# jshi31/T2ONet

Hardware: AMD Instinct MI355X
Metric: images/sec (train step: episode forward + END select + L1 + backward + gradient all-reduce + Adam, bs=64/GPU, 256x256 fp32) (higher is better)
Workload: dtype f32; 1 GPU; BASELINE.json configs[2]: full T2ONet episode/L1 train step (train_seq2seqL1.py:74-88), bs=64 per GPU, 256x256 fp32, FiveK-shaped synthetic batch, random-init weights; global_batch=64, parallelism=dp1: batch shards, one flat fp32 gradient all-reduce (22.2 M floats) per step, world_size=1

## Files before the change

### include/t2onet_hip.h

```cpp
#ifndef T2ONET_HIP_H
#define T2ONET_HIP_H

#include <stddef.h>

#ifdef __cplusplus
extern "C" {
#endif

#define T2O_OK 0
#define T2O_EINVAL 1
#define T2O_EUNSUPPORTED 2
#define T2O_EWORKSPACE 3
#define T2O_ELAUNCH 4

#define T2O_OP_IDENTITY (-1)
#define T2O_MAX_PARAM 24

int t2o_abi_version(void);
const char* t2o_last_error(void);
const char* t2o_source_digest(void);

int t2o_op_num_params(int op);

size_t t2o_workspace_bytes(int B, int H, int W);
// ... 164 lines not shown


int t2o_bn_relu_nhwc_bwd_acc(const float* x, const float* y, const float* dy, const float* weight, const float* bias,
                             const float* save_mean, const float* save_invstd, float* dx, float* dres, float* dweight,
                             float* dbias, int has_res, int relu, int accumulate, void* workspace, size_t workspace_bytes,
                             int M, int C, void* stream);
int t2o_bn_relu_nhwc_bwd_partials_acc(const float* x, const float* dy, const float* weight, const float* bias,
                                      const float* save_mean, const float* save_invstd, float* dx, float* dweight,
                                      float* dbias, int relu, int accumulate, const float* partial, int partial_rows,
                                      void* workspace, size_t workspace_bytes, int M, int C, void* stream);

int t2o_conv3x3_wgrad_acc_nhwc(const float* x, const float* dy, float* dw, void* workspace, size_t workspace_bytes,
                               int N, int Ho, int Wo, int Ci, int Co, int stride, int accumulate, void* stream);

int t2o_conv_weight_transform(const float* w, float* wt, int Co, int Ci, int taps, int flip, void* stream);
int t2o_conv_weight_transform_batch(const float* const* w, float* const* wt, const int* Co, const int* Ci, const int* taps,
                                    const int* flip, int n, void* stream);

int t2o_conv3x3_dgrad_pre_nhwc(const float* dy, const float* wt, const float* addend, float* dx, void* workspace,
                               size_t workspace_bytes, int N, int H, int W, int Ci, int Co, void* stream);
int t2o_conv3x3_dgrad_bnsums_rows(int N, int H, int W, int Ci, int Co);
int t2o_conv3x3_dgrad_pre_bnsums_nhwc(const float* dy, const float* wt, float* dx, const float* bn_x,
                                      const float* save_mean, const float* save_invstd, const float* weight,
                                      const float* bias, float* rows, void* workspace, size_t workspace_bytes,
                                      int N, int H, int W, int Ci, int Co, void* stream);
int t2o_conv3x3s2_dgrad_pre_nhwc(const float* dy, const float* wt, float* dx, void* workspace, size_t workspace_bytes,
                                 int N, int Ho, int Wo, int Ci, int Co, void* stream);

int t2o_stem_fwd(const float* x, const float* w, float* y, float* stats, int N, int Ho, int Wo, int Co, int planar, void* stream);
int t2o_stem_fwd_any(const float* x, const float* w, float* y, float* stats, int N, int Hi, int Wi, int Co, int planar, void* stream);
int t2o_stem_wgrad(const float* x, const float* dy, float* dw, void* workspace, size_t workspace_bytes, int N, int Ho, int Wo,
                   int Co, int planar, int accumulate, void* stream);
int t2o_stem_dgrad(const float* dy, const float* w, float* dx, int N, int Ho, int Wo, int Co, int planar, int accumulate, void* stream);

int t2o_conv1x1s2_fwd_nhwc(const float* x, const float* w, float* y, int N, int H, int W, int Ci, int Co, void* stream);
int t2o_conv1x1s2_dgrad_acc_nhwc(const float* dy, const float* wt, float* dx, int N, int H, int W, int Ci, int Co, void* stream);
size_t t2o_conv1x1s2_wgrad_workspace_bytes(int N, int H, int W, int Ci, int Co);
int t2o_conv1x1s2_wgrad_nhwc(const float* x, const float* dy, float* dw, void* workspace, size_t workspace_bytes,
                             int N, int H, int W, int Ci, int Co, int accumulate, void* stream);

int t2o_conv3x3_any_fwd_nhwc(const float* x, const float* w, float* y, int N, int H, int W, int Ci, int Co, int stride, void* stream);
int t2o_conv3x3_any_dgrad_nhwc(const float* dy, const float* wt, const float* addend, float* dx, int N, int H, int W, int Ci, int Co,
                               int stride, void* stream);
size_t t2o_conv3x3_any_wgrad_workspace_bytes(int N, int H, int W, int Ci, int Co, int stride);
int t2o_conv3x3_any_wgrad_nhwc(const float* x, const float* dy, float* dw, void* workspace, size_t workspace_bytes,
                               int N, int H, int W, int Ci, int Co, int stride, int accumulate, void* stream);

int t2o_wino_padded_tiles(int N, int H, int W);
int t2o_wino_weight_transform(const float* w, float* U, int Cn, int Ck, void* stream);
int t2o_wino_weight_transform_batch(const float* const* w, float* const* U, const int* Cn, const int* Ck, int n, void* stream);
int t2o_wino_weight_transform_chunked_batch(const float* const* w, float* const* Uc, const int* Cn, const int* Ck, int n, void* stream);
int t2o_wino_input_transform(const float* x, float* V, int N, int H, int W, int C, void* stream);
int t2o_wino_input_transform_ld(const float* x, float* V, int N, int H, int W, int C, int plane_rows, void* stream);
int t2o_wino_stats_rows(int N, int H, int W, int C);
int t2o_wino_output_transform(const float* M, const float* addend, float* y, float* stats, int N, int H, int W, int C, void* stream);
int t2o_wino_dy_transform(const float* dy, float* Ad, int N, int H, int W, int C, void* stream);
int t2o_wino_dy_transforms(const float* dy, float* V, float* Ad, int N, int H, int W, int C, void* stream);
int t2o_wino_dy_transforms_ld(const float* dy, float* V, float* Ad, int N, int H, int W, int C, int ad_plane_rows, void* stream);
int t2o_wino_dy_transform_ld(const float* dy, float* Ad, int N, int H, int W, int C, int plane_rows, void* stream);
int t2o_wino_dw_transform(const float* dU, float* dw, int Co, int Ci, int splits, int accumulate, void* stream);
int t2o_gemm_nt_batched(const float* A, const float* B, float* C, int batches, int M, int N, int K, int a_rows, void* stream);
int t2o_gemm_tn_splits(int batches, int rows, int M, int N);
int t2o_gemm_tn_batched(const float* A, const float* B, float* C, int batches, int rows, int M, int N, int splits, void* stream);
int t2o_gemm_tn_batched_ld(const float* A, const float* B, float* C, int batches, int rows, int a_plane_rows, int b_plane_rows, int M, int N,
                           int splits, void* stream);

// ... 125 lines not shown
```

### t2onet_amd/_lib.py

```python
import ctypes
import os

import torch

_HERE = os.path.dirname(os.path.abspath(__file__))
LIB_PATH = os.path.join(_HERE, 'lib', 'libt2onet_hip.so')

c_f = ctypes.POINTER(ctypes.c_float)
c_i = ctypes.POINTER(ctypes.c_int)
_P = ctypes.c_void_p
_I = ctypes.c_int
_Z = ctypes.c_size_t
_F = ctypes.c_float
_D = ctypes.c_double

SIGNATURES = {
    't2o_abi_version': (_I, []),
    't2o_last_error': (ctypes.c_char_p, []),
    't2o_source_digest': (ctypes.c_char_p, []),
    't2o_op_num_params': (_I, [_I]),
    't2o_workspace_bytes': (_Z, [_I, _I, _I]),
    't2o_op_fwd': (_I, [_I, _P, _P, _I, _P, _I, _P, _I, _I, _I, _P]),
    't2o_op_bwd': (_I, [_I, _P, _P, _I, _P, _I, _P, _P, _P, _I, _P, _Z, _I, _I, _I, _P]),
    't2o_apply_fwd': (_I, [_P, _P, _P, _I, _P, _I, _P, _I, _I, _I, _P]),
# ... 69 lines not shown
    't2o_wino_weight_transform_chunked_batch': (_I, [_P, _P, _P, _P, _I, _P]),
    't2o_end_select_l1_fwd': (_I, [_P, _I, _P, _P, _P, _I, _Z, _P, _Z, _P]),
    't2o_end_select_l1_bwd': (_I, [_P, _P, _I, _P, _P, _P, _I, _Z, _P]),
    't2o_wino_padded_tiles': (_I, [_I, _I, _I]),
    't2o_wino_weight_transform': (_I, [_P, _P, _I, _I, _P]),
    't2o_gemm_nt_batched': (_I, [_P, _P, _P, _I, _I, _I, _I, _I, _P]),
    't2o_gemm': (_I, [_P, _P, _P, _I, _I, _I, _I, _I, _I, _I, _I, _I, _P]),
    't2o_colsum': (_I, [_P, _P, _I, _I, _I, _I, _P]),
    't2o_gemm_tn_splits': (_I, [_I, _I, _I, _I]),
    't2o_gemm_tn_batched': (_I, [_P, _P, _P, _I, _I, _I, _I, _I, _P]),
    't2o_gemm_tn_batched_ld': (_I, [_P, _P, _P, _I, _I, _I, _I, _I, _I, _I, _P]),
    't2o_wino_input_transform': (_I, [_P, _P, _I, _I, _I, _I, _P]),
    't2o_wino_input_transform_ld': (_I, [_P, _P, _I, _I, _I, _I, _I, _P]),
    't2o_wino_stats_rows': (_I, [_I, _I, _I, _I]),
    't2o_wino_output_transform': (_I, [_P, _P, _P, _P, _I, _I, _I, _I, _P]),
    't2o_wino_dy_transform': (_I, [_P, _P, _I, _I, _I, _I, _P]),
    't2o_wino_dy_transforms': (_I, [_P, _P, _P, _I, _I, _I, _I, _P]),
    't2o_wino_dy_transforms_ld': (_I, [_P, _P, _P, _I, _I, _I, _I, _I, _P]),
    't2o_wino_dy_transform_ld': (_I, [_P, _P, _I, _I, _I, _I, _I, _P]),
    't2o_wino_dw_transform': (_I, [_P, _P, _I, _I, _I, _I, _P]),
    't2o_conv3x3_dgrad_pre_nhwc': (_I, [_P, _P, _P, _P, _P, _Z, _I, _I, _I, _I, _I, _P]),
    't2o_conv3x3_dgrad_bnsums_rows': (_I, [_I, _I, _I, _I, _I]),
    't2o_wino_fused_supported': (_I, [_I, _I, _I, _I, _I]),
    't2o_wino_fused_stats_rows': (_I, [_I, _I, _I]),
    't2o_wino_u_chunked': (_I, [_P, _P, _I, _I, _P]),
    't2o_wino_fused_conv_nhwc': (_I, [_P, _P, _P, _P, _P, _P, _I, _I, _I, _I, _I, _P]),
    't2o_wino_fused_conv_bnsums_nhwc': (_I, [_P, _P, _P, _P, _P, _P, _P, _P, _P, _P, _I, _I, _I, _I, _I, _P]),
    't2o_conv3x3_dgrad_pre_bnsums_nhwc': (_I, [_P, _P, _P, _P, _P, _P, _P, _P, _P, _P, _Z, _I, _I, _I, _I, _I, _P]),
    't2o_conv3x3s2_dgrad_pre_nhwc': (_I, [_P, _P, _P, _P, _Z, _I, _I, _I, _I, _I, _P]),
    't2o_stem_fwd': (_I, [_P, _P, _P, _P, _I, _I, _I, _I, _I, _P]),
    't2o_stem_fwd_any': (_I, [_P, _P, _P, _P, _I, _I, _I, _I, _I, _P]),
    't2o_stem_wgrad': (_I, [_P, _P, _P, _P, _Z, _I, _I, _I, _I, _I, _I, _P]),
    't2o_stem_dgrad': (_I, [_P, _P, _P, _I, _I, _I, _I, _I, _I, _P]),
    't2o_conv1x1s2_fwd_nhwc': (_I, [_P, _P, _P, _I, _I, _I, _I, _I, _P]),
    't2o_conv1x1s2_dgrad_acc_nhwc': (_I, [_P, _P, _P, _I, _I, _I, _I, _I, _P]),
    't2o_conv1x1s2_wgrad_workspace_bytes': (_Z, [_I, _I, _I, _I, _I]),
    't2o_conv1x1s2_wgrad_nhwc': (_I, [_P, _P, _P, _P, _Z, _I, _I, _I, _I, _I, _I, _P]),
    't2o_fused_sequence_prepare': (_I, [_P, _I]),
    't2o_jit_set_cache_dir': (_I, [ctypes.c_char_p]),
    't2o_jit_specialisations': (_I, []),
    't2o_conv3x3_any_fwd_nhwc': (_I, [_P, _P, _P, _I, _I, _I, _I, _I, _I, _P]),
    't2o_conv3x3_any_dgrad_nhwc': (_I, [_P, _P, _P, _P, _I, _I, _I, _I, _I, _I, _P]),
    't2o_conv3x3_any_wgrad_workspace_bytes': (_Z, [_I, _I, _I, _I, _I, _I]),
    't2o_conv3x3_any_wgrad_nhwc': (_I, [_P, _P, _P, _P, _Z, _I, _I, _I, _I, _I, _I, _I, _P]),
    't2o_lstm_layer_fwd': (_I, [_P, _P, _P, _P, _P, _P, _P, _P, _P, _I, _I, _I, _I, _P]),
    't2o_lstm_layer_bwd': (_I, [_P, _P, _P, _P, _P, _P, _P, _P, _P, _P, _I, _I, _I, _I, _P]),
    't2o_bn_dual_nhwc_workspace_bytes': (_Z, [_I, _I]),
    't2o_bn_dual_relu_nhwc_fwd': (_I, [_P, _P, _I, _P] + [_P] * 13 + [_F, _F, _F, _F, _P, _Z, _I, _I, _P]),
    't2o_bn_dual_relu_nhwc_bwd_acc': (_I, [_P] * 18 + [_I, _P, _Z, _I, _I, _P]),
    't2o_image_feature_fwd': (_I, [_P, _P]),
    't2o_image_feature_bwd': (_I, [_P, _P]),
    't2o_decoder_step_fwd': (_I, [_P, _P]),
    't2o_decoder_step_bwd': (_I, [_P, _P]),
    't2o_resize_u8_to_f32': (_I, [_P, _P, _I, _I, _I, _P, _P]),
    't2o_f32_to_u8_hwc': (_I, [_P, _I, _I, _I, _P, _P]),
    't2o_replay_u8': (_I, [_P, _P, _P, _I, _P, _P]),
    't2o_replay_u8_masked': (_I, [_P, _P, _P, _P, _I, _P, _P, _P, _I, _P]),
    't2o_eval_metrics_workspace_bytes': (_Z, [_I, _I, _I, _I]),
    't2o_eval_metrics': (_I, [_P, _P, _I, _P, _P, _P, _I, _P, _Z, _I, _I, _I, _I, _P]),
    't2o_end_select_var_mean_workspace_bytes': (_Z, [_Z]),
    't2o_end_select_var_mean': (_I, [_P, _P, _I, _I, _I, _Z, _P, _P, _Z, _P]),
}


class ImageFeatureArgs(ctypes.Structure):
    _fields_ = ([(n, _P) for n in ('fc_w', 'fc_b', 'bn_w', 'bn_b', 'running_mean', 'running_var', 'num_batches_tracked', 'pooled',
# ... 57 lines not shown
```

### t2onet_amd/build.py

```python
import fcntl
import hashlib
import os
import subprocess
import sys

HERE = os.path.dirname(os.path.abspath(__file__))
ROOT = os.path.dirname(HERE)
CSRC = os.path.join(HERE, 'csrc')
LIBDIR = os.path.join(HERE, 'lib')
LIB = os.path.join(LIBDIR, 'libt2onet_hip.so')
SOURCES = ['t2o_stamp.hip', 't2o_kernels.hip', 't2o_jit.hip', 't2o_norm.hip', 't2o_conv.hip', 't2o_conv1x1.hip', 't2o_conv_generic.hip', 't2o_winograd.hip', 't2o_wino_fused.hip', 't2o_wino_wgrad.hip', 't2o_gemm.hip', 't2o_rnn.hip', 't2o_decoder.hip', 't2o_heads.hip', 't2o_optim.hip', 't2o_planner_fit.hip', 't2o_image_io.hip', 't2o_replay.hip', 't2o_replay_mask.hip', 't2o_eval.hip', 't2o_comm.hip']
HEADERS = ['t2o_pixel_math.h', 't2o_image_math.h', 't2o_replay_math.h', 't2o_replay_mask_math.h', 't2o_eval_math.h', 't2o_block_programs.h', 't2o_chain_kernels.h', 't2o_jit.h', os.path.join(ROOT, 'include', 't2onet_hip.h')]
ARCH = 'gfx950'
FLAGS = ['-O3', '--offload-arch=' + ARCH, '-DT2O_ARCH="%s"' % ARCH, '-ffp-contract=off', '-std=c++17', '-fPIC', '-shared',
         '-I' + os.path.join(ROOT, 'include'), '-I' + os.path.join(HERE, 'lib'), '-ldl']
OBJDIR = os.path.join(LIBDIR, 'obj')
JIT_HEADERS = ['t2o_pixel_math.h', 't2o_image_math.h', 't2o_block_programs.h', 't2o_chain_kernels.h']


def write_embedded_headers():
    parts = ['// generated by t2onet_amd/build.py from csrc/*.h -- do not edit\n',
             'static const int kJitHeaderCount = %d;\n' % len(JIT_HEADERS),
             'static const char* kJitHeaderNames[] = {%s};\n' % ', '.join('"%s"' % h for h in JIT_HEADERS),
             'static const char* kJitHeaderSources[] = {\n']
    for h in JIT_HEADERS:
        with open(os.path.join(CSRC, h)) as f:
            text = f.read()
        assert ')T2OJIT"' not in text
        pieces = [text[i:i + 16000] for i in range(0, len(text), 16000)]
        parts.append(' '.join('R"T2OJIT(%s)T2OJIT"' % p for p in pieces) + ',\n')
    parts.append('};\n')
    out = ''.join(parts)
    path = os.path.join(LIBDIR, 't2o_jit_embedded.h')
    try:
        with open(path) as f:
            if f.read() == out:
                return
    except OSError:
        pass
    with open(path, 'w') as f:
        f.write(out)


def hipcc_path():
# ... 129 lines not shown
```

### t2onet_amd/csrc/t2o_norm.hip

```cpp
#include <hip/hip_runtime.h>

#include "t2onet_hip.h"

namespace {

constexpr int kThreads = 256;
constexpr int kUnroll = 4;

struct BnArgs {
  const float* x;
  const float* res;
  const float* dy;
  const float* y;
  float* out;
  float* dres;
  const float* weight;
  const float* bias;
  float* running_mean;
  float* running_var;
  float* save_mean;
  float* save_invstd;
  float* coef;
  float* dweight;
  float* dbias;
// ... 722 lines not shown
  const size_t total4 = (size_t)M * (C >> 2);
  const unsigned grid = flat_grid(total4, 1, kUnroll);
  if (res) k_bn_nhwc_apply<true><<<grid, kThreads, 0, st>>>(a, total4); else k_bn_nhwc_apply<false><<<grid, kThreads, 0, st>>>(a, total4);
  return hipGetLastError() == hipSuccess ? T2O_OK : set_error(T2O_ELAUNCH, "batch-norm kernel launch failed");
}

int t2o_bn_relu_nhwc_bwd_acc(const float* x, const float* y, const float* dy, const float* weight, const float* bias,
                             const float* save_mean, const float* save_invstd, float* dx, float* dres, float* dweight,
                             float* dbias, int has_res, int relu, int accumulate, void* workspace, size_t workspace_bytes,
                             int M, int C, void* stream) {
  if (!x || M <= 0 || !nhwc_channels_ok(C) || !dy || !weight || !bias || !save_mean || !save_invstd || !dx)
    return set_error(T2O_EINVAL, "bn_relu_nhwc_bwd: null pointer or bad shape (C must be a power of two in [4, 1024])");
  if (has_res && relu && !y) return set_error(T2O_EINVAL, "bn_relu_nhwc_bwd: y is needed when a residual was added");
  if (!workspace || workspace_bytes < t2o_bn_nhwc_workspace_bytes(M, C)) return set_error(T2O_EWORKSPACE, "bn_relu_nhwc_bwd: workspace too small");
  BnArgs a = {};
  a.x = x; a.y = y; a.dy = dy; a.out = dx; a.dres = dres; a.weight = weight; a.bias = bias;
  a.save_mean = const_cast<float*>(save_mean); a.save_invstd = const_cast<float*>(save_invstd);
  a.dweight = dweight; a.dbias = dbias;
  a.N = M; a.C = C; a.HW = 1; a.splits = 1; a.relu = relu; a.acc = accumulate ? 1 : 0;
  a.partials = (double*)workspace;
  a.coef = (float*)((char*)workspace + sizeof(double) * 2 * (size_t)C);
  float* partial = a.coef + 4 * (size_t)C;
  hipStream_t st = (hipStream_t)stream;
  int rpb, nblk;
  nhwc_partition(M, C, 2, &rpb, &nblk);
  if (has_res) k_bn_nhwc_bwd_sums<true><<<nblk, kThreads, 0, st>>>(a, M, rpb, partial); else k_bn_nhwc_bwd_sums<false><<<nblk, kThreads, 0, st>>>(a, M, rpb, partial);
  k_bn_nhwc_finalize<true><<<C / 4, kThreads, 0, st>>>(a, partial, nblk);
  const size_t total4 = (size_t)M * (C >> 2);
  const unsigned grid = flat_grid(total4, 1, 2);
  if (has_res) k_bn_nhwc_bwd_apply<true><<<grid, kThreads, 0, st>>>(a, total4); else k_bn_nhwc_bwd_apply<false><<<grid, kThreads, 0, st>>>(a, total4);
  return hipGetLastError() == hipSuccess ? T2O_OK : set_error(T2O_ELAUNCH, "batch-norm kernel launch failed");
}

int t2o_bn_relu_nhwc_bwd_partials_acc(const float* x, const float* dy, const float* weight, const float* bias,
                                      const float* save_mean, const float* save_invstd, float* dx, float* dweight, float* dbias,
                                      int relu, int accumulate, const float* partial, int partial_rows, void* workspace,
                                      size_t workspace_bytes, int M, int C, void* stream) {
  if (!x || M <= 0 || !nhwc_channels_ok(C) || !dy || !weight || !bias || !save_mean || !save_invstd || !dx)
    return set_error(T2O_EINVAL, "bn_relu_nhwc_bwd_partials: null pointer or bad shape (C must be a power of two in [4, 1024])");
  if (!partial || partial_rows <= 0) return set_error(T2O_EINVAL, "bn_relu_nhwc_bwd_partials: no partial sums");
  if (!workspace || workspace_bytes < t2o_bn_nhwc_workspace_bytes(M, C)) return set_error(T2O_EWORKSPACE, "bn_relu_nhwc_bwd_partials: workspace too small");
  BnArgs a = {};
  a.x = x; a.dy = dy; a.out = dx; a.weight = weight; a.bias = bias;
  a.save_mean = const_cast<float*>(save_mean); a.save_invstd = const_cast<float*>(save_invstd);
  a.dweight = dweight; a.dbias = dbias;
  a.N = M; a.C = C; a.HW = 1; a.splits = 1; a.relu = relu; a.acc = accumulate ? 1 : 0;
  a.partials = (double*)workspace;
  a.coef = (float*)((char*)workspace + sizeof(double) * 2 * (size_t)C);
  hipStream_t st = (hipStream_t)stream;
  k_bn_nhwc_finalize<true><<<C / 4, kThreads, 0, st>>>(a, partial, partial_rows);
  const size_t total4 = (size_t)M * (C >> 2);
  k_bn_nhwc_bwd_apply<false><<<flat_grid(total4, 1, 2), kThreads, 0, st>>>(a, total4);
  return hipGetLastError() == hipSuccess ? T2O_OK : set_error(T2O_ELAUNCH, "batch-norm kernel launch failed");
}

int t2o_bn_relu_nhwc_bwd(const float* x, const float* y, const float* dy, const float* weight, const float* bias,
                         const float* save_mean, const float* save_invstd, float* dx, float* dres, float* dweight,
                         float* dbias, int has_res, int relu, void* workspace, size_t workspace_bytes, int M, int C,
                         void* stream) {
  return t2o_bn_relu_nhwc_bwd_acc(x, y, dy, weight, bias, save_mean, save_invstd, dx, dres, dweight, dbias, has_res, relu, 0,
                                  workspace, workspace_bytes, M, C, stream);
}

size_t t2o_bn_dual_nhwc_workspace_bytes(int M, int C) {
  (void)M;
  return sizeof(float) * 8 * (size_t)C + sizeof(float) * 3 * (size_t)C * kNhwcMaxBlocks + sizeof(float) * 2 * (size_t)C * kNhwcMaxBlocks;
// ... 75 lines not shown
```

### t2onet_amd/encoder.py

```python
import os

import torch

from . import _lib
from .functional import (_need_gpu, _persistent_grad, _ptr, _stream, _conv_workspace, _zero_block, wino_conv_nhwc, wino_fused_conv_nhwc, wino_wgrad_nhwc, wino_input,
                         wino_backward_nhwc, wino_dw_from, wino_fused_wgrad_nhwc)

_WINOGRAD = os.environ.get('T2O_WINOGRAD', '1') != '0'
_WINO_MIN_C = int(os.environ.get('T2O_WINOGRAD_MIN_C', '256'))
_DUAL_BN = True
_WINO_FUSED = os.environ.get('T2O_WINOGRAD_FUSED', '1') != '0'
_BN_SUMS_EPILOGUE = True
_WINO_WGRAD = os.environ.get('T2O_WINOGRAD_WGRAD', '1') != '0'


def _fast_direct(stride, Hi, Wi, Wo):
    return Wo % 8 == 0 and (stride == 1 or (Hi % 2 == 0 and Wi % 2 == 0))


def _batched(fn, name, st, srcs, dsts, int_lists):
    import ctypes
    for i in range(0, len(srcs), 32):
        n = min(32, len(srcs) - i)
        a = (ctypes.c_void_p * n)(*[t.data_ptr() for t in srcs[i:i + n]])
        b = (ctypes.c_void_p * n)(*[t.data_ptr() for t in dsts[i:i + n]])
        ints = [(ctypes.c_int * n)(*lst[i:i + n]) for lst in int_lists]
        _lib.check(fn(a, b, *ints, n, st), name)


def _nhwc(N, H, W, C, dev):
    return torch.empty((N, H, W, C), dtype=torch.float32, device=dev)


class TrunkPlan:

    def __init__(self, resnet):
        self.net = resnet
        blocks = [b for layer in (resnet.layer1, resnet.layer2, resnet.layer3, resnet.layer4) for b in layer]
        self.blocks = blocks
        self.params = [resnet.conv1.weight, resnet.bn1.weight, resnet.bn1.bias]
        self.index = {}
        for b in blocks:
            self.params += [b.conv1.weight, b.bn1.weight, b.bn1.bias, b.conv2.weight, b.bn2.weight, b.bn2.bias]
            if len(b.shortcut):
# ... 583 lines not shown
                rc = lib.t2o_bn_relu_nhwc_bwd_partials_acc(_ptr(rec['y1']), _ptr(da1), _ptr(b.bn1.weight), _ptr(b.bn1.bias), _ptr(rec['m1']),
                                                           _ptr(rec['i1']), _ptr(dy1), _ptr(g(b.bn1.weight)), _ptr(g(b.bn1.bias)), 1, acc,
                                                           _ptr(rows1), rows1.numel() // (2 * Co), _ptr(bn_ws), bn_ws.numel(), M, Co, st)
                _lib.check(rc, 't2o_bn_relu_nhwc_bwd_partials_acc')
            else:
                dy1, _ = bn_bwd(b.bn1, rec['y1'], None, da1, rec['m1'], rec['i1'], 0, 1, False, M, Co, slot1)
            del da1
            dx = torch.empty_like(rec['x'])
            if plan.wino(b.conv1, Hc, Wc) and not len(b.shortcut) and plan.kernel_for(b.conv1, N, Hc, Wc, 'wgrad') != 'wino_wgrad':
                wino_bwd(b.conv1, rec['x'], dy1, dx, dsc, Hc, Wc)
                d = dx
                continue
            if slot1 is None:
                wgrad3(b.conv1, rec['x'], dy1, Hc, Wc, Hn, Wn)
            if len(b.shortcut):
                sc_conv, sc_bn = b.shortcut[0], b.shortcut[1]
                if dys is None:
                    slots = deferred(sc_conv)
                    dys, _ = bn_bwd(sc_bn, rec['ys'], None, dsc, rec['ms'], rec['is_'], 0, 0, False, M, Co, slots)
                if slots is None:
                    need = lib.t2o_conv1x1s2_wgrad_workspace_bytes(N, Hc, Wc, Ci, Co)
                    ws = torch.empty(need, dtype=torch.uint8, device=dev)
                    rc = lib.t2o_conv1x1s2_wgrad_nhwc(_ptr(rec['x']), _ptr(dys), _ptr(g(sc_conv.weight)), _ptr(ws), need, N, Hc, Wc, Ci, Co,
                                                      acc, st)
                    _lib.check(rc, 't2o_conv1x1s2_wgrad_nhwc')
                dgrad3(b.conv1, dy1, dx, None, Hc, Wc, Hn, Wn)
                rc = lib.t2o_conv1x1s2_dgrad_acc_nhwc(_ptr(dys), _ptr(wt[id(sc_conv)]), _ptr(dx), N, Hc, Wc, Ci, Co, st)
                _lib.check(rc, 't2o_conv1x1s2_dgrad_acc_nhwc')
            else:
                dgrad3(b.conv1, dy1, dx, dsc, Hc, Wc, Hn, Wn)
            d = dx
        y0, m0, i0 = ctx.stem
        _, Ho, Wo, C0 = y0.shape
        dy0, _ = bn_bwd(net.bn1, y0, None, d, m0, i0, 0, 1, False, N * Ho * Wo, C0)
        need = lib.t2o_stem_wgrad_workspace_bytes(N, Ho, Wo, C0)
        ws = torch.empty(need, dtype=torch.uint8, device=dev)
        rc = lib.t2o_stem_wgrad(_ptr(ctx.img), _ptr(dy0), _ptr(g(net.conv1.weight)), _ptr(ws), need, N, Ho, Wo, C0, ctx.planar, acc, st)
        _lib.check(rc, 't2o_stem_wgrad')
        dimg = None
        if ctx.needs_input_grad[1]:
            dimg = torch.empty_like(ctx.img)
            rc = lib.t2o_stem_dgrad(_ptr(dy0), _ptr(net.conv1.weight), _ptr(dimg), N, Ho, Wo, C0, ctx.planar, 0, st)
            _lib.check(rc, 't2o_stem_dgrad')
        if arena is not None:
            arena.done.add(apass)
        return (None, dimg) + (tuple(None for _ in plan.params) if acc else tuple(grads))


def trunk_forward(plan, img, pool=False):
    plan.pool = bool(pool)
    return _TrunkFn.apply(plan, img, *plan.params)
```

### t2onet_amd/functional.py

```python
import ctypes

import os

import numpy as np
import torch

from . import _lib

OP_NPARAM = (1, 1, 1, 24, 1, 8, 1, 1)
PARAM_PAD = 24
_workspaces = {}


_raw_stream = getattr(torch._C, '_cuda_getCurrentRawStream', None)


def _stream(device=None):
    if _raw_stream is not None:
        return _raw_stream(torch.cuda.current_device() if device is None or device.index is None else device.index)
    return torch.cuda.current_stream(device).cuda_stream


def _ptr(t):
    return None if t is None else t.data_ptr()
# ... 1047 lines not shown
    dw = into if into is not None else torch.empty((Co, Ci, 1, 1), dtype=torch.float32, device=x.device)
    rc = lib.t2o_conv1x1s2_wgrad_nhwc(_ptr(x), _ptr(dy), _ptr(dw), _ptr(ws), need, N, H, W, Ci, Co, 1 if into is not None else 0,
                                      _stream(x.device))
    _lib.check(rc, 't2o_conv1x1s2_wgrad_nhwc')
    return dw


def stem_planar(x, weight, dy=None, want='fwd', into=None):
    lib = _lib.load()
    Co = weight.shape[0]
    w = weight.contiguous(memory_format=torch.channels_last)
    if want == 'dgrad':
        N, _, Ho, Wo = dy.shape
        dy = dy.contiguous(memory_format=torch.channels_last)
        dx = into if into is not None else torch.empty((N, 3, 2 * Ho, 2 * Wo), dtype=torch.float32, device=dy.device)
        _lib.check(lib.t2o_stem_dgrad(_ptr(dy), _ptr(w), _ptr(dx), N, Ho, Wo, Co, 1, 1 if into is not None else 0, _stream(dy.device)),
                   't2o_stem_dgrad')
        return dx
    x = x.contiguous()
    N, _, Hi, Wi = x.shape
    Ho, Wo = Hi // 2, Wi // 2
    if want == 'fwd':
        y = torch.empty((N, Co, Ho, Wo), dtype=torch.float32, device=x.device, memory_format=torch.channels_last)
        stats = torch.empty((lib.t2o_stem_fwd_stats_rows(N, Ho, Wo), 2, Co), dtype=torch.float32, device=x.device)
        _lib.check(lib.t2o_stem_fwd(_ptr(x), _ptr(w), _ptr(y), _ptr(stats), N, Ho, Wo, Co, 1, _stream(x.device)), 't2o_stem_fwd')
        return y, stats
    dy = dy.contiguous(memory_format=torch.channels_last)
    need = lib.t2o_stem_wgrad_workspace_bytes(N, Ho, Wo, Co)
    ws = torch.empty(need, dtype=torch.uint8, device=x.device)
    dw = into if into is not None else torch.empty((Co, 3, 3, 3), dtype=torch.float32, device=x.device, memory_format=torch.channels_last)
    _lib.check(lib.t2o_stem_wgrad(_ptr(x), _ptr(dy), _ptr(dw), _ptr(ws), need, N, Ho, Wo, Co, 1, 1 if into is not None else 0,
                                  _stream(x.device)), 't2o_stem_wgrad')
    return dw


def _ld(t, what):
    if t.dim() != 2 or t.dtype != torch.float32 or (t.shape[1] > 1 and t.stride(1) != 1) or t.stride(0) < t.shape[1]:
        raise ValueError('%s must be a 2-D fp32 matrix with contiguous rows (a column slice of a larger one is fine)' % what)
    return t.stride(0)


def gemm(A, B, out=None, a_kmajor=False, b_kmajor=False, accumulate=False):
    _need_gpu(A, B)
    K, M = (A.shape[0], A.shape[1]) if a_kmajor else (A.shape[1], A.shape[0])
    Kb, N = (B.shape[0], B.shape[1]) if b_kmajor else (B.shape[1], B.shape[0])
    if K != Kb:
        raise ValueError('gemm: contraction lengths differ (%d vs %d)' % (K, Kb))
    if out is None:
        if accumulate:
            raise ValueError('gemm: accumulate needs `out`')
        out = torch.empty((M, N), dtype=torch.float32, device=A.device)
    elif tuple(out.shape) != (M, N):
        raise ValueError('gemm: out is %s, the product (%d, %d)' % (tuple(out.shape), M, N))
    if M == 0 or N == 0:
        return out
    if K == 0:
        return out if accumulate else out.zero_()
    rc = _lib.load().t2o_gemm(_ptr(A), _ptr(B), _ptr(out), M, N, K, _ld(A, 'gemm: A'), _ld(B, 'gemm: B'), _ld(out, 'gemm: out'),
                              1 if a_kmajor else 0, 1 if b_kmajor else 0, 1 if accumulate else 0, _stream(A.device))
    _lib.check(rc, 't2o_gemm')
    return out


def colsum(X, out=None, accumulate=False):
    _need_gpu(X)
    R, N = X.shape
# ... 673 lines not shown
```

Measured before the change: 1860 images/sec.

## Fuse stem batch-norm backward with stem weight and input gradients

Replaces the stem's separate BN backward (which wrote a full dy0 tensor) plus the stem wgrad and dgrad kernels. A coefficient-only BN backward pass now computes the per-channel reduction terms, and new fused kernels recompute dy0 on the fly from y0 and the upstream gradient inside the wgrad/dgrad tiles. This removes one full-resolution write and two reads of the dy0 intermediate at 128x128x32/64 per image. In exchange, dy0 is recomputed in both kernels under default form 1, and the new kernels carry a large register footprint.

Result: no change. 1864 images/sec (median of 5 runs) (+0.2%).

```diff
diff --git a/include/t2onet_hip.h b/include/t2onet_hip.h
--- a/include/t2onet_hip.h
+++ b/include/t2onet_hip.h
@@ -220,6 +220,13 @@
 int t2o_stem_wgrad(const float* x, const float* dy, float* dw, void* workspace, size_t workspace_bytes, int N, int Ho, int Wo,
                    int Co, int planar, int accumulate, void* stream);
 int t2o_stem_dgrad(const float* dy, const float* w, float* dx, int N, int Ho, int Wo, int Co, int planar, int accumulate, void* stream);
+
+int t2o_bn_relu_nhwc_bwd_coef_acc(const float* x, const float* dy, const float* weight, const float* bias, const float* save_mean,
+                                  const float* save_invstd, float* dweight, float* dbias, float* coef, int relu, int accumulate,
+                                  void* workspace, size_t workspace_bytes, int M, int C, void* stream);
+int t2o_stem_bwd_fused(const float* x, const float* y0, const float* d, const float* w, const float* bn_bias, const float* save_mean,
+                       const float* save_invstd, const float* coef, float* dw, float* dx, void* workspace, size_t workspace_bytes,
+                       int N, int Ho, int Wo, int Co, int planar, int accumulate, int dx_accumulate, int form, void* stream);
 
 int t2o_conv1x1s2_fwd_nhwc(const float* x, const float* w, float* y, int N, int H, int W, int Ci, int Co, void* stream);
 int t2o_conv1x1s2_dgrad_acc_nhwc(const float* dy, const float* wt, float* dx, int N, int H, int W, int Ci, int Co, void* stream);
diff --git a/t2onet_amd/_lib.py b/t2onet_amd/_lib.py
--- a/t2onet_amd/_lib.py
+++ b/t2onet_amd/_lib.py
@@ -125,6 +125,8 @@
     't2o_stem_fwd_any': (_I, [_P, _P, _P, _P, _I, _I, _I, _I, _I, _P]),
     't2o_stem_wgrad': (_I, [_P, _P, _P, _P, _Z, _I, _I, _I, _I, _I, _I, _P]),
     't2o_stem_dgrad': (_I, [_P, _P, _P, _I, _I, _I, _I, _I, _I, _P]),
+    't2o_bn_relu_nhwc_bwd_coef_acc': (_I, [_P, _P, _P, _P, _P, _P, _P, _P, _P, _I, _I, _P, _Z, _I, _I, _P]),
+    't2o_stem_bwd_fused': (_I, [_P, _P, _P, _P, _P, _P, _P, _P, _P, _P, _P, _Z, _I, _I, _I, _I, _I, _I, _I, _I, _P]),
     't2o_conv1x1s2_fwd_nhwc': (_I, [_P, _P, _P, _I, _I, _I, _I, _I, _P]),
     't2o_conv1x1s2_dgrad_acc_nhwc': (_I, [_P, _P, _P, _I, _I, _I, _I, _I, _P]),
     't2o_conv1x1s2_wgrad_workspace_bytes': (_Z, [_I, _I, _I, _I, _I]),
diff --git a/t2onet_amd/build.py b/t2onet_amd/build.py
--- a/t2onet_amd/build.py
+++ b/t2onet_amd/build.py
@@ -9,7 +9,7 @@
 CSRC = os.path.join(HERE, 'csrc')
 LIBDIR = os.path.join(HERE, 'lib')
 LIB = os.path.join(LIBDIR, 'libt2onet_hip.so')
-SOURCES = ['t2o_stamp.hip', 't2o_kernels.hip', 't2o_jit.hip', 't2o_norm.hip', 't2o_conv.hip', 't2o_conv1x1.hip', 't2o_conv_generic.hip', 't2o_winograd.hip', 't2o_wino_fused.hip', 't2o_wino_wgrad.hip', 't2o_gemm.hip', 't2o_rnn.hip', 't2o_decoder.hip', 't2o_heads.hip', 't2o_optim.hip', 't2o_planner_fit.hip', 't2o_image_io.hip', 't2o_replay.hip', 't2o_replay_mask.hip', 't2o_eval.hip', 't2o_comm.hip']
+SOURCES = ['t2o_stamp.hip', 't2o_kernels.hip', 't2o_jit.hip', 't2o_norm.hip', 't2o_conv.hip', 't2o_stem_bwd.hip', 't2o_conv1x1.hip', 't2o_conv_generic.hip', 't2o_winograd.hip', 't2o_wino_fused.hip', 't2o_wino_wgrad.hip', 't2o_gemm.hip', 't2o_rnn.hip', 't2o_decoder.hip', 't2o_heads.hip', 't2o_optim.hip', 't2o_planner_fit.hip', 't2o_image_io.hip', 't2o_replay.hip', 't2o_replay_mask.hip', 't2o_eval.hip', 't2o_comm.hip']
 HEADERS = ['t2o_pixel_math.h', 't2o_image_math.h', 't2o_replay_math.h', 't2o_replay_mask_math.h', 't2o_eval_math.h', 't2o_block_programs.h', 't2o_chain_kernels.h', 't2o_jit.h', os.path.join(ROOT, 'include', 't2onet_hip.h')]
 ARCH = 'gfx950'
 FLAGS = ['-O3', '--offload-arch=' + ARCH, '-DT2O_ARCH="%s"' % ARCH, '-ffp-contract=off', '-std=c++17', '-fPIC', '-shared',
diff --git a/t2onet_amd/csrc/t2o_norm.hip b/t2onet_amd/csrc/t2o_norm.hip
--- a/t2onet_amd/csrc/t2o_norm.hip
+++ b/t2onet_amd/csrc/t2o_norm.hip
@@ -778,6 +778,28 @@
   return hipGetLastError() == hipSuccess ? T2O_OK : set_error(T2O_ELAUNCH, "batch-norm kernel launch failed");
 }
 
+int t2o_bn_relu_nhwc_bwd_coef_acc(const float* x, const float* dy, const float* weight, const float* bias, const float* save_mean,
+                                  const float* save_invstd, float* dweight, float* dbias, float* coef, int relu, int accumulate,
+                                  void* workspace, size_t workspace_bytes, int M, int C, void* stream) {
+  if (!x || M <= 0 || !nhwc_channels_ok(C) || !dy || !weight || !bias || !save_mean || !save_invstd || !coef)
+    return set_error(T2O_EINVAL, "bn_relu_nhwc_bwd_coef: null pointer or bad shape (C must be a power of two in [4, 1024])");
+  if (!workspace || workspace_bytes < t2o_bn_nhwc_workspace_bytes(M, C)) return set_error(T2O_EWORKSPACE, "bn_relu_nhwc_bwd_coef: workspace too small");
+  BnArgs a = {};
+  a.x = x; a.dy = dy; a.weight = weight; a.bias = bias;
+  a.save_mean = const_cast<float*>(save_mean); a.save_invstd = const_cast<float*>(save_invstd);
+  a.dweight = dweight; a.dbias = dbias;
+  a.N = M; a.C = C; a.HW = 1; a.splits = 1; a.relu = relu; a.acc = accumulate ? 1 : 0;
+  a.partials = (double*)workspace;
+  a.coef = coef;
+  float* partial = (float*)((char*)workspace + sizeof(double) * 2 * (size_t)C) + 4 * (size_t)C;
+  hipStream_t st = (hipStream_t)stream;
+  int rpb, nblk;
+  nhwc_partition(M, C, 2, &rpb, &nblk);
+  k_bn_nhwc_bwd_sums<false><<<nblk, kThreads, 0, st>>>(a, M, rpb, partial);
+  k_bn_nhwc_finalize<true><<<C / 4, kThreads, 0, st>>>(a, partial, nblk);
+  return hipGetLastError() == hipSuccess ? T2O_OK : set_error(T2O_ELAUNCH, "batch-norm kernel launch failed");
+}
+
 int t2o_bn_relu_nhwc_bwd_partials_acc(const float* x, const float* dy, const float* weight, const float* bias,
                                       const float* save_mean, const float* save_invstd, float* dx, float* dweight, float* dbias,
                                       int relu, int accumulate, const float* partial, int partial_rows, void* workspace,
diff --git a/t2onet_amd/csrc/t2o_stem_bwd.hip b/t2onet_amd/csrc/t2o_stem_bwd.hip
--- /dev/null
+++ b/t2onet_amd/csrc/t2o_stem_bwd.hip
@@ -0,0 +1,345 @@
+#include <hip/hip_runtime.h>
+
+#include <cstdint>
+
+#include "t2onet_hip.h"
+
+namespace t2o {
+int set_error(int code, const char* msg);
+void launch_wgrad_reduce(const float* partial, float* dw, size_t n, int splits, int accumulate, hipStream_t st);
+}
+using t2o::set_error;
+
+namespace {
+
+constexpr int kTH = 8, kTW = 32;
+constexpr int kPix = (kTH + 1) * (kTW + 1);
+constexpr int kPlane = kPix + 1;
+constexpr int kRows = 2 * kTH + 1, kRowPix = 2 * kTW + 1, kRowFloats = kRowPix * 3;
+constexpr int kTilesPerWg = 8;
+
+struct StemBwdArgs {
+  const float* x;
+  const float* y0;
+  const float* d;
+  const float* w;
+  const float* bias;
+  const float* mean;
+  const float* invstd;
+  const float* coef;
+  float* partial;
+  float* dx;
+  int N, Ho, Wo, tiles_total, acc_dx;
+};
+
+__device__ __forceinline__ float4 ldg4(const float* p) { return *reinterpret_cast<const float4*>(p); }
+
+struct BnCoef { float4 mean, invstd, ac, mg, mgx, sh; };
+
+template <int kCo>
+__device__ __forceinline__ BnCoef load_coef(const StemBwdArgs& a, int cq) {
+  BnCoef c;
+  c.mean = ldg4(a.mean + 4 * cq); c.invstd = ldg4(a.invstd + 4 * cq);
+  const float4 bi = ldg4(a.bias + 4 * cq);
+  c.ac = ldg4(a.coef + 4 * cq); c.mg = ldg4(a.coef + kCo + 4 * cq); c.mgx = ldg4(a.coef + 2 * kCo + 4 * cq);
+  c.sh = make_float4(bi.x - c.mean.x * c.ac.x, bi.y - c.mean.y * c.ac.y, bi.z - c.mean.z * c.ac.z, bi.w - c.mean.w * c.ac.w);
+  return c;
+}
+
+__device__ __forceinline__ float dy_of(float y, float d, float ac, float sh, float mg, float mean, float invstd, float mgx) {
+  const float g = (y * ac + sh > 0.0f) ? d : 0.0f;
+  return ac * ((g - mg) - ((y - mean) * invstd) * mgx);
+}
+
+__device__ __forceinline__ float4 dy_of4(const float4 y, const float4 d, const BnCoef& c) {
+  return make_float4(dy_of(y.x, d.x, c.ac.x, c.sh.x, c.mg.x, c.mean.x, c.invstd.x, c.mgx.x),
+                     dy_of(y.y, d.y, c.ac.y, c.sh.y, c.mg.y, c.mean.y, c.invstd.y, c.mgx.y),
+                     dy_of(y.z, d.z, c.ac.z, c.sh.z, c.mg.z, c.mean.z, c.invstd.z, c.mgx.z),
+                     dy_of(y.w, d.w, c.ac.w, c.sh.w, c.mg.w, c.mean.w, c.invstd.w, c.mgx.w));
+}
+
+template <int kUnroll, class Plane>
+__device__ __forceinline__ void dgrad_quads(float (&acc)[2][2][3], Plane plane, int nq, int p00, const float* __restrict__ w, int c_first) {
+#pragma unroll kUnroll
+  for (int cq = 0; cq < nq; ++cq) {
+    const float4* t = plane(cq);
+    const float4 d00 = t[p00], d01 = t[p00 + 1], d10 = t[p00 + kTW + 1], d11 = t[p00 + kTW + 2];
+    const float v00[4] = {d00.x, d00.y, d00.z, d00.w}, v01[4] = {d01.x, d01.y, d01.z, d01.w};
+    const float v10[4] = {d10.x, d10.y, d10.z, d10.w}, v11[4] = {d11.x, d11.y, d11.z, d11.w};
+#pragma unroll
+    for (int k = 0; k < 4; ++k) {
+      const float* wc = w + (size_t)(c_first + cq * 4 + k) * 27;
+#pragma unroll
+      for (int kh = 0; kh < 3; ++kh)
+#pragma unroll
+        for (int kw = 0; kw < 3; ++kw) {
+          const int ph = kh != 1, pw = kw != 1;
+          const float d = kh == 0 ? (kw == 0 ? v11[k] : v10[k]) : (kw == 0 ? v01[k] : v00[k]);
+#pragma unroll
+          for (int c = 0; c < 3; ++c) acc[ph][pw][c] = fmaf(d, wc[(kh * 3 + kw) * 3 + c], acc[ph][pw][c]);
+        }
+    }
+  }
+}
+
+template <bool kPlanar>
+__device__ __forceinline__ void dgrad_store(const float (&acc)[2][2][3], float* __restrict__ dx, int n, int al, int be, int Ho, int Wo, int acc_out) {
+  if (al < Ho && be < Wo) {
+    if constexpr (kPlanar) {
+#pragma unroll
+      for (int c = 0; c < 3; ++c)
+#pragma unroll
+        for (int ph = 0; ph < 2; ++ph) {
+          float2* o = reinterpret_cast<float2*>(dx + (((size_t)n * 3 + c) * 2 * Ho + 2 * al + ph) * 2 * Wo + 2 * be);
+          float2 v = make_float2(acc[ph][0][c], acc[ph][1][c]);
+          if (acc_out) { const float2 u = *o; v.x += u.x; v.y += u.y; }
+          *o = v;
+        }
+    } else {
+#pragma unroll
+      for (int ph = 0; ph < 2; ++ph) {
+        float* o = dx + ((((size_t)n * 2 * Ho + 2 * al + ph) * 2 * Wo) + 2 * be) * 3;
+#pragma unroll
+        for (int q = 0; q < 6; ++q) o[q] = acc_out ? o[q] + acc[ph][q / 3][q % 3] : acc[ph][q / 3][q % 3];
+      }
+    }
+  }
+}
+
+template <int kCo, bool kPlanar, bool kDgrad>
+__global__ __launch_bounds__(256, kDgrad ? 1 : 2) void k_stem_bwd(StemBwdArgs a) {
+  constexpr int kThreads = 256;
+  constexpr int kUnroll = kDgrad ? 2 : 1;
+  constexpr int CQ = kCo / 4, PP = 256 / CQ, kPasses = (kTH * kTW) / PP;
+  __shared__ __attribute__((aligned(16))) float patch[kRows][kRowFloats + 1];
+  __shared__ float red[PP][kCo + 1];
+  __shared__ float4 tile[kDgrad ? CQ : 1][kDgrad ? kPlane : 1];
+  const int tid = threadIdx.x;
+  const int Ho = a.Ho, Wo = a.Wo, Hi = 2 * Ho, Wi = 2 * Wo;
+  const int tiles_w = (Wo + kTW - 1) / kTW, tiles_h = (Ho + kTH - 1) / kTH;
+  const int cq = tid % CQ, ps = tid / CQ;
+  __shared__ float4 cf[6][CQ];
+  if (tid < CQ) {
+    const BnCoef c = load_coef<kCo>(a, tid);
+    cf[0][tid] = c.mean; cf[1][tid] = c.invstd; cf[2][tid] = c.ac; cf[3][tid] = c.mg; cf[4][tid] = c.mgx; cf[5][tid] = c.sh;
+  }
+  __syncthreads();
+  auto coefs = [&]() {
+    __asm__ volatile("" ::: "memory");
+    BnCoef c;
+    c.mean = cf[0][cq]; c.invstd = cf[1][cq]; c.ac = cf[2][cq]; c.mg = cf[3][cq]; c.mgx = cf[4][cq]; c.sh = cf[5][cq];
+    return c;
+  };
+  float acc[4][27];
+#pragma unroll
+  for (int j = 0; j < 4; ++j)
+#pragma unroll
+    for (int t = 0; t < 27; ++t) acc[j][t] = 0.0f;
+
+  constexpr int kLoadsX = (kRows * kRowFloats + kThreads - 1) / kThreads;
+  constexpr int kLoadsD = kDgrad ? (kPix * CQ + kThreads - 1) / kThreads : 1;
+  float stage[kLoadsX];
+  float4 sy[kLoadsD], sd[kLoadsD];
+  auto issue = [&](int tile_i) {
+    const int n = tile_i / (tiles_h * tiles_w), th = (tile_i / tiles_w) % tiles_h, tw = tile_i % tiles_w;
+    const int ih0 = 2 * th * kTH - 1, iw0 = 2 * tw * kTW - 1;
+#pragma unroll
+    for (int k = 0; k < kLoadsX; ++k) {
+      int f = tid + kThreads * k;
+      if constexpr (kDgrad) __asm__ volatile("" : "+v"(f));
+      const int rr = f / kRowFloats, cc = f - rr * kRowFloats;
+      if constexpr (kPlanar) {
+        const int ci = cc / kRowPix, ih = ih0 + rr, iw = iw0 + (cc - ci * kRowPix);
+        stage[k] = (f < kRows * kRowFloats && ih >= 0 && ih < Hi && iw >= 0 && iw < Wi) ? a.x[(((size_t)n * 3 + ci) * Hi + ih) * Wi + iw] : 0.0f;
+      } else {
+        const int ih = ih0 + rr, iw = iw0 + cc / 3;
+        stage[k] = (f < kRows * kRowFloats && ih >= 0 && ih < Hi && iw >= 0 && iw < Wi) ? a.x[(((size_t)n * Hi + ih) * Wi + iw0) * 3 + cc] : 0.0f;
+      }
+    }
+    if constexpr (kDgrad) {
+      const int a0 = th * kTH, b0 = tw * kTW;
+#pragma unroll
+      for (int k = 0; k < kLoadsD; ++k) {
+        int f = tid + kThreads * k;
+        __asm__ volatile("" : "+v"(f));
+        const int px = f / CQ;
+        const int sa = a0 + px / (kTW + 1), sb = b0 + px % (kTW + 1);
+        const bool in = f < kPix * CQ && sa < Ho && sb < Wo;
+        const size_t off = (((size_t)n * Ho + sa) * Wo + sb) * kCo + 4 * cq;
+        sy[k] = in ? ldg4(a.y0 + off) : make_float4(0.0f, 0.0f, 0.0f, 0.0f);
+        sd[k] = in ? ldg4(a.d + off) : make_float4(0.0f, 0.0f, 0.0f, 0.0f);
+      }
+    }
+  };
+
+  const int tile0 = blockIdx.x * kTilesPerWg;
+  if (tile0 < a.tiles_total) issue(tile0);
+  for (int tt = 0; tt < kTilesPerWg; ++tt) {
+    const int tile_i = tile0 + tt;
+    if (tile_i >= a.tiles_total) break;
+    const int n = tile_i / (tiles_h * tiles_w), th = (tile_i / tiles_w) % tiles_h, tw = tile_i % tiles_w;
+    const int a0 = th * kTH, b0 = tw * kTW;
+    if (tt) __syncthreads();
+#pragma unroll
+    for (int k = 0; k < kLoadsX; ++k) {
+      int f = tid + kThreads * k;
+      if constexpr (kDgrad) __asm__ volatile("" : "+v"(f));
+      const int rr = f / kRowFloats, cc = f - rr * kRowFloats;
+      const int pc = kPlanar ? (cc % kRowPix) * 3 + cc / kRowPix : cc;
+      if (f < kRows * kRowFloats) patch[rr][pc] = stage[k];
+    }
+    if constexpr (kDgrad) {
+      const BnCoef co = coefs();
+#pragma unroll
+      for (int k = 0; k < kLoadsD; ++k) {
+        int f = tid + kThreads * k;
+        __asm__ volatile("" : "+v"(f));
+        const int px = f / CQ;
+        const int sa = a0 + px / (kTW + 1), sb = b0 + px % (kTW + 1);
+        if (f < kPix * CQ) tile[cq][px] = (sa < Ho && sb < Wo) ? dy_of4(sy[k], sd[k], co) : make_float4(0.0f, 0.0f, 0.0f, 0.0f);
+      }
+    }
+    __syncthreads();
+    if (tt + 1 < kTilesPerWg && tile_i + 1 < a.tiles_total) issue(tile_i + 1);
+    {
+      float4 yq = make_float4(0.0f, 0.0f, 0.0f, 0.0f), gq = yq;
+      auto fetch = [&](int pass) {
+        const int pix = pass * PP + ps, oh = a0 + pix / kTW, ow = b0 + pix % kTW;
+        if (oh < Ho && ow < Wo) {
+          const size_t off = (((size_t)n * Ho + oh) * Wo + ow) * kCo + 4 * cq;
+          yq = ldg4(a.y0 + off); gq = ldg4(a.d + off);
+        }
+      };
+      if constexpr (!kDgrad) fetch(0);
+#pragma unroll kUnroll
+      for (int pass = 0; pass < kPasses; ++pass) {
+        const int pix = pass * PP + ps, r = pix / kTW, c = pix % kTW;
+        float4 dq;
+        if constexpr (kDgrad) {
+          dq = tile[cq][r * (kTW + 1) + c];
+        } else {
+          dq = make_float4(0.0f, 0.0f, 0.0f, 0.0f);
+          if (a0 + r < Ho && b0 + c < Wo) dq = dy_of4(yq, gq, coefs());
+          if (pass + 1 < kPasses) fetch(pass + 1);
+        }
+        const float dv[4] = {dq.x, dq.y, dq.z, dq.w};
+#pragma unroll
+        for (int kh = 0; kh < 3; ++kh) {
+          const float* row = &patch[2 * r + kh][6 * c];
+#pragma unroll
+          for (int t = 0; t < 9; ++t) {
+            const float xv = row[t];
+#pragma unroll
+            for (int j = 0; j < 4; ++j) acc[j][kh * 9 + t] = fmaf(dv[j], xv, acc[j][kh * 9 + t]);
+          }
+        }
+      }
+    }
+    if constexpr (kDgrad) {
+      const int ta = tid / kTW, tbeta = tid % kTW;
+      float ax[2][2][3] = {};
+      dgrad_quads<kUnroll>(ax, [&](int q) { return &tile[q][0]; }, CQ, ta * (kTW + 1) + tbeta, a.w, 0);
+      dgrad_store<kPlanar>(ax, a.dx, n, a0 + ta, b0 + tbeta, Ho, Wo, a.acc_dx);
+    }
+  }
+  float* out = a.partial + (size_t)blockIdx.x * kCo * 27;
+#pragma unroll
+  for (int t = 0; t < 27; ++t) {
+    __syncthreads();
+#pragma unroll
+    for (int j = 0; j < 4; ++j) red[ps][4 * cq + j] = acc[j][t];
+    __syncthreads();
+    if (tid < kCo) {
+      float sum = 0.0f;
+      for (int k = 0; k < PP; ++k) sum += red[k][tid];
+      out[tid * 27 + t] = sum;
+    }
+  }
+}
+
+static_assert(((kPix * 8 + 255) / 256) % 2 == 0, "k_stem_bwd_dgrad stages its tile in two equal rounds");
+
+template <int kCo, bool kPlanar>
+__global__ __launch_bounds__(256) void k_stem_bwd_dgrad(StemBwdArgs a) {
+  constexpr int kPass = 32, CQ = kPass / 4;
+  __shared__ float4 tile[CQ][kPlane];
+  const int Ho = a.Ho, Wo = a.Wo;
+  const int tiles_w = (Wo + kTW - 1) / kTW, tiles_h = (Ho + kTH - 1) / kTH;
+  const int tb = blockIdx.x;
+  const int n = tb / (tiles_h * tiles_w), th = (tb / tiles_w) % tiles_h, tw = tb % tiles_w;
+  const int a0 = th * kTH, b0 = tw * kTW;
+  const int ta = threadIdx.x / kTW, tbeta = threadIdx.x % kTW;
+  const int cq = threadIdx.x % CQ;
+  float acc[2][2][3] = {};
+  for (int c0 = 0; c0 < kCo; c0 += kPass) {
+    if (c0) __syncthreads();
+    const BnCoef co = load_coef<kCo>(a, c0 / 4 + cq);
+    constexpr int kLoads = (kPix * CQ + 255) / 256, kHalf = kLoads / 2;
+#pragma unroll
+    for (int k0 = 0; k0 < kLoads; k0 += kHalf) {
+      float4 sy[kHalf], sd[kHalf];
+#pragma unroll
+      for (int k = 0; k < kHalf; ++k) {
+        const int f = threadIdx.x + 256 * (k0 + k);
+        const int px = f / CQ;
+        const int sa = a0 + px / (kTW + 1), sb = b0 + px % (kTW + 1);
+        const bool in = f < kPix * CQ && sa < Ho && sb < Wo;
+        const size_t off = (((size_t)n * Ho + sa) * Wo + sb) * kCo + c0 + 4 * cq;
+        sy[k] = in ? ldg4(a.y0 + off) : make_float4(0.0f, 0.0f, 0.0f, 0.0f);
+        sd[k] = in ? ldg4(a.d + off) : make_float4(0.0f, 0.0f, 0.0f, 0.0f);
+      }
+#pragma unroll
+      for (int k = 0; k < kHalf; ++k) {
+        const int f = threadIdx.x + 256 * (k0 + k);
+        const int px = f / CQ;
+        const int sa = a0 + px / (kTW + 1), sb = b0 + px % (kTW + 1);
+        if (f < kPix * CQ) tile[cq][px] = (sa < Ho && sb < Wo) ? dy_of4(sy[k], sd[k], co) : make_float4(0.0f, 0.0f, 0.0f, 0.0f);
+      }
+    }
+    __syncthreads();
+    dgrad_quads<2>(acc, [&](int q) { return &tile[q][0]; }, CQ, ta * (kTW + 1) + tbeta, a.w, c0);
+  }
+  dgrad_store<kPlanar>(acc, a.dx, n, a0 + ta, b0 + tbeta, Ho, Wo, a.acc_dx);
+}
+
+template <int kCo, bool kPlanar>
+void launch(const StemBwdArgs& a, int rows, int form, hipStream_t st) {
+  if (!a.dx) { k_stem_bwd<kCo, kPlanar, false><<<(unsigned)rows, 256, 0, st>>>(a); return; }
+  if (form == 0) { k_stem_bwd<kCo, kPlanar, true><<<(unsigned)rows, 256, 0, st>>>(a); return; }
+  k_stem_bwd<kCo, kPlanar, false><<<(unsigned)rows, 256, 0, st>>>(a);
+  k_stem_bwd_dgrad<kCo, kPlanar><<<(unsigned)a.tiles_total, 256, 0, st>>>(a);
+}
+
+bool aligned(const void* p, uintptr_t n) { return ((uintptr_t)p & (n - 1)) == 0; }
+
+}
+
+extern "C" {
+
+int t2o_stem_bwd_fused(const float* x, const float* y0, const float* d, const float* w, const float* bn_bias, const float* save_mean,
+                       const float* save_invstd, const float* coef, float* dw, float* dx, void* workspace, size_t workspace_bytes,
+                       int N, int Ho, int Wo, int Co, int planar, int accumulate, int dx_accumulate, int form, void* stream) {
+  if (!x || !y0 || !d || !w || !bn_bias || !save_mean || !save_invstd || !coef || !dw) return set_error(T2O_EINVAL, "stem_bwd_fused: null pointer");
+  if (!aligned(x, 4) || !aligned(w, 4) || !aligned(y0, 16) || !aligned(d, 16) || !aligned(bn_bias, 16) || !aligned(save_mean, 16) ||
+      !aligned(save_invstd, 16) || !aligned(coef, 16) || !aligned(dw, 16) || !aligned(dx, planar ? 8 : 4) || !aligned(workspace, 16))
+    return set_error(T2O_EINVAL, "stem_bwd_fused: misaligned pointer (16 bytes: y0, d, the batch-norm vectors, dw, workspace; 8: a planar dx)");
+  if (N <= 0 || Ho <= 0 || Wo <= 0 || (Co != 32 && Co != 64)) return set_error(T2O_EUNSUPPORTED, "stem_bwd_fused: 3 input channels, 32 or 64 output channels");
+  if (form != 0 && form != 1) return set_error(T2O_EINVAL, "stem_bwd_fused: form is 0 (one kernel) or 1 (two kernels)");
+  const long long tiles = (long long)N * ((Ho + kTH - 1) / kTH) * ((Wo + kTW - 1) / kTW);
+  if (tiles >= ((long long)1 << 30)) return set_error(T2O_EUNSUPPORTED, "stem_bwd_fused: too many tiles");
+  if (dx && (size_t)N * Ho * Wo * 4 >= ((size_t)1 << 31)) return set_error(T2O_EUNSUPPORTED, "stem_bwd_fused: image gradient too large");
+  const size_t need = t2o_stem_wgrad_workspace_bytes(N, Ho, Wo, Co);
+  if (!workspace || workspace_bytes < need) return set_error(T2O_EWORKSPACE, "stem_bwd_fused: workspace too small");
+  const int rows = t2o_stem_fwd_stats_rows(N, Ho, Wo);
+  StemBwdArgs a = {};
+  a.x = x; a.y0 = y0; a.d = d; a.w = w; a.bias = bn_bias; a.mean = save_mean; a.invstd = save_invstd; a.coef = coef;
+  a.partial = (float*)workspace; a.dx = dx;
+  a.N = N; a.Ho = Ho; a.Wo = Wo; a.tiles_total = (int)tiles; a.acc_dx = dx_accumulate ? 1 : 0;
+  hipStream_t st = (hipStream_t)stream;
+  if (Co == 64) { if (planar) launch<64, true>(a, rows, form, st); else launch<64, false>(a, rows, form, st); }
+  else { if (planar) launch<32, true>(a, rows, form, st); else launch<32, false>(a, rows, form, st); }
+  t2o::launch_wgrad_reduce(a.partial, dw, (size_t)Co * 27, rows, accumulate, st);
+  return hipGetLastError() == hipSuccess ? T2O_OK : set_error(T2O_ELAUNCH, "stem_bwd_fused launch failed");
+}
+
+}
diff --git a/t2onet_amd/encoder.py b/t2onet_amd/encoder.py
--- a/t2onet_amd/encoder.py
+++ b/t2onet_amd/encoder.py
@@ -3,6 +3,7 @@
 import torch
 
 from . import _lib
+from . import functional as _F
 from .functional import (_need_gpu, _persistent_grad, _ptr, _stream, _conv_workspace, _zero_block, wino_conv_nhwc, wino_fused_conv_nhwc, wino_wgrad_nhwc, wino_input,
                          wino_backward_nhwc, wino_dw_from, wino_fused_wgrad_nhwc)
 
@@ -10,6 +11,7 @@
 _WINO_MIN_C = int(os.environ.get('T2O_WINOGRAD_MIN_C', '256'))
 _DUAL_BN = True
 _WINO_FUSED = os.environ.get('T2O_WINOGRAD_FUSED', '1') != '0'
+_STEM_BWD_FUSED = os.environ.get('T2O_STEM_BWD_FUSED', '1') != '0'
 _BN_SUMS_EPILOGUE = True
 _WINO_WGRAD = os.environ.get('T2O_WINOGRAD_WGRAD', '1') != '0'
 
@@ -659,16 +661,28 @@
             d = dx
         y0, m0, i0 = ctx.stem
         _, Ho, Wo, C0 = y0.shape
-        dy0, _ = bn_bwd(net.bn1, y0, None, d, m0, i0, 0, 1, False, N * Ho * Wo, C0)
         need = lib.t2o_stem_wgrad_workspace_bytes(N, Ho, Wo, C0)
         ws = torch.empty(need, dtype=torch.uint8, device=dev)
-        rc = lib.t2o_stem_wgrad(_ptr(ctx.img), _ptr(dy0), _ptr(g(net.conv1.weight)), _ptr(ws), need, N, Ho, Wo, C0, ctx.planar, acc, st)
-        _lib.check(rc, 't2o_stem_wgrad')
         dimg = None
         if ctx.needs_input_grad[1]:
             dimg = torch.empty_like(ctx.img)
-            rc = lib.t2o_stem_dgrad(_ptr(dy0), _ptr(net.conv1.weight), _ptr(dimg), N, Ho, Wo, C0, ctx.planar, 0, st)
-            _lib.check(rc, 't2o_stem_dgrad')
+        if _STEM_BWD_FUSED:
+            bn = net.bn1
+            coef = torch.empty((3, C0), dtype=torch.float32, device=dev)
+            rc = lib.t2o_bn_relu_nhwc_bwd_coef_acc(_ptr(y0), _ptr(d), _ptr(bn.weight), _ptr(bn.bias), _ptr(m0), _ptr(i0), _ptr(g(bn.weight)),
+                                                   _ptr(g(bn.bias)), _ptr(coef), 1, acc, _ptr(bn_ws), bn_ws.numel(), N * Ho * Wo, C0, st)
+            _lib.check(rc, 't2o_bn_relu_nhwc_bwd_coef_acc')
+            rc = lib.t2o_stem_bwd_fused(_ptr(ctx.img), _ptr(y0), _ptr(d), _ptr(net.conv1.weight), _ptr(bn.bias), _ptr(m0), _ptr(i0), _ptr(coef),
+                                        _ptr(g(net.conv1.weight)), _ptr(dimg), _ptr(ws), need, N, Ho, Wo, C0, ctx.planar, acc, 0,
+                                        _F._STEM_BWD_FORM, st)
+            _lib.check(rc, 't2o_stem_bwd_fused')
+        else:
+            dy0, _ = bn_bwd(net.bn1, y0, None, d, m0, i0, 0, 1, False, N * Ho * Wo, C0)
+            rc = lib.t2o_stem_wgrad(_ptr(ctx.img), _ptr(dy0), _ptr(g(net.conv1.weight)), _ptr(ws), need, N, Ho, Wo, C0, ctx.planar, acc, st)
+            _lib.check(rc, 't2o_stem_wgrad')
+            if dimg is not None:
+                rc = lib.t2o_stem_dgrad(_ptr(dy0), _ptr(net.conv1.weight), _ptr(dimg), N, Ho, Wo, C0, ctx.planar, 0, st)
+                _lib.check(rc, 't2o_stem_dgrad')
         if arena is not None:
             arena.done.add(apass)
         return (None, dimg) + (tuple(None for _ in plan.params) if acc else tuple(grads))
diff --git a/t2onet_amd/functional.py b/t2onet_amd/functional.py
--- a/t2onet_amd/functional.py
+++ b/t2onet_amd/functional.py
@@ -1103,6 +1103,46 @@
     _lib.check(lib.t2o_stem_wgrad(_ptr(x), _ptr(dy), _ptr(dw), _ptr(ws), need, N, Ho, Wo, Co, 1, 1 if into is not None else 0,
                                   _stream(x.device)), 't2o_stem_wgrad')
     return dw
+
+
+_STEM_BWD_FORM = 1
+
+
+def stem_backward_fused(x, y0, d, weight, bn_weight, bn_bias, save_mean, save_invstd, dw=None, dgamma=None, dbeta=None,
+                        accumulate=False, want_dx=True, dx=None, form=None):
+    _need_gpu(x, y0, d, weight)
+    lib = _lib.load()
+    dev = y0.device
+    st = _stream(dev)
+    N, Co, Ho, Wo = y0.shape
+    if tuple(x.shape) != (N, 3, 2 * Ho, 2 * Wo) or tuple(d.shape) != tuple(y0.shape) or Co not in (32, 64):
+        raise ValueError('stem_backward_fused: x must be (N, 3, 2 Ho, 2 Wo), y0 and d (N, Co, Ho, Wo) with 32 or 64 channels')
+    planar = 1 if x.is_contiguous() else 0
+    if not planar:
+        x = x.contiguous(memory_format=torch.channels_last)
+    y0 = y0.contiguous(memory_format=torch.channels_last)
+    d = d.contiguous(memory_format=torch.channels_last)
+    weight = weight.contiguous(memory_format=torch.channels_last)
+    if dw is None:
+        dw = torch.empty((Co, 3, 3, 3), dtype=torch.float32, device=dev, memory_format=torch.channels_last)
+    dgamma = torch.empty(Co, dtype=torch.float32, device=dev) if dgamma is None else dgamma
+    dbeta = torch.empty(Co, dtype=torch.float32, device=dev) if dbeta is None else dbeta
+    acc = 1 if accumulate else 0
+    coef = torch.empty((3, Co), dtype=torch.float32, device=dev)
+    bn_ws = torch.empty(lib.t2o_bn_nhwc_workspace_bytes(N * Ho * Wo, Co), dtype=torch.uint8, device=dev)
+    rc = lib.t2o_bn_relu_nhwc_bwd_coef_acc(_ptr(y0), _ptr(d), _ptr(bn_weight), _ptr(bn_bias), _ptr(save_mean), _ptr(save_invstd),
+                                           _ptr(dgamma), _ptr(dbeta), _ptr(coef), 1, acc, _ptr(bn_ws), bn_ws.numel(), N * Ho * Wo, Co, st)
+    _lib.check(rc, 't2o_bn_relu_nhwc_bwd_coef_acc')
+    dx_acc = 1 if dx is not None else 0
+    if dx is None and want_dx:
+        dx = torch.empty_like(x)
+    need = lib.t2o_stem_wgrad_workspace_bytes(N, Ho, Wo, Co)
+    ws = torch.empty(need, dtype=torch.uint8, device=dev)
+    rc = lib.t2o_stem_bwd_fused(_ptr(x), _ptr(y0), _ptr(d), _ptr(weight), _ptr(bn_bias), _ptr(save_mean), _ptr(save_invstd), _ptr(coef),
+                                _ptr(dw), _ptr(dx), _ptr(ws), need, N, Ho, Wo, Co, planar, acc, dx_acc,
+                                _STEM_BWD_FORM if form is None else form, st)
+    _lib.check(rc, 't2o_stem_bwd_fused')
+    return dw, dgamma, dbeta, dx
 
 
 def _ld(t, what):
```
